# zju3dv/OnePose_Plus_Plus

Hardware: AMD Instinct MI355X
Metric: query images/sec (2D-3D match fwd) at 512x512 img x 5k pts (higher is better)
Workload: dtype f32 (operands as exact bf16 triples, f32 accumulate)

## Files before the change

### include/opp_hip.h

```cpp
#ifndef OPP_HIP_H
#define OPP_HIP_H

#include <stddef.h>

#ifdef __cplusplus
extern "C" {
#endif

#define OPP_MAX_LAYERS 16

typedef struct opp_config {
  int initial_dim;
  int block_dims[3];
  int kpt_enc_enable;
  int kpt_enc_dims[3];
  int pos_enc_enable;
  int coarse_d_model;
  int coarse_nhead;
  int coarse_n_layers;
  int coarse_is_cross[OPP_MAX_LAYERS];
  int fine_d_model;
  int fine_nhead;
  int fine_n_layers;
  int fine_is_cross[OPP_MAX_LAYERS];
// ... 31 lines not shown
                     size_t packed_bytes, void* stream);
int opp_set_pack_scope(opp_ctx* ctx, int scope);

int opp_num_bn_layers(const opp_ctx* ctx);
const char* opp_bn_layer_name(const opp_ctx* ctx, int i);
int opp_bn_layer_channels(const opp_ctx* ctx, int i);
size_t opp_packed_train_weights_bytes(const opp_ctx* ctx);
int opp_pack_train_weights(opp_ctx* ctx, const float* const* weights, int n_weights, void* packed,
                           size_t packed_bytes, void* stream);
size_t opp_backbone_train_workspace_bytes(const opp_ctx* ctx, int B, int H, int W);
int opp_backbone_train(opp_ctx* ctx, const float* image, int B, int H, int W, float* feat_c, float* feat_f,
                       float* bn_stats, void* workspace, size_t workspace_bytes, void* stream);

size_t opp_backbone_workspace_bytes(const opp_ctx* ctx, int H, int W);
int opp_backbone(opp_ctx* ctx, const float* image, int H, int W, float* feat_c, float* feat_f,
                 void* workspace, size_t workspace_bytes, void* stream);

int opp_coarse_tokens(opp_ctx* ctx, const float* feat_c, const float* pe, int L, const float* kpts,
                      const float* bank_c, int n_points, float* tokens, void* workspace,
                      size_t workspace_bytes, void* stream);

int opp_encode_points(opp_ctx* ctx, const float* kpts, const float* bank_c, int n_points,
                      float* tokens3d, void* workspace, size_t workspace_bytes, void* stream);

size_t opp_object_prefix_bytes(const opp_ctx* ctx, int n_points);
size_t opp_object_prefix_workspace_bytes(const opp_ctx* ctx, int n_points);
int opp_object_prefix(opp_ctx* ctx, const float* tokens3d, int n_points, void* prefix, size_t prefix_bytes, void* workspace,
                      size_t workspace_bytes, void* stream);
int opp_set_object_prefix(opp_ctx* ctx, const void* prefix, int n_points);

size_t opp_transformer_workspace_bytes(const opp_ctx* ctx, int which, int n_seg, int len0, int len1);
int opp_transformer(opp_ctx* ctx, int which, float* tokens, int n_seg, int len0, int len1,
                    void* workspace, size_t workspace_bytes, void* stream);

size_t opp_coarse_match_workspace_bytes(const opp_ctx* ctx, int n_points, int L);
int opp_coarse_match(opp_ctx* ctx, const float* feat3d, const float* feat2d, int n_points, int hc,
                     int wc, const float* kpts, float base_scale, const float* query_scale, float* conf,
                     long long* i_ids, long long* j_ids, float* mconf, float* mkpts_c,
                     float* mkpts_3d, int* count, void* workspace, size_t workspace_bytes,
                     void* stream);

size_t opp_forward_coarse_workspace_bytes(const opp_ctx* ctx, int H, int W, int n_points);
int opp_forward_coarse(opp_ctx* ctx, const float* image, int H, int W, const float* pe,
                       const float* kpts, const float* bank_c, const float* tokens3d_pre, int n_points,
                       float base_scale, const float* query_scale, float* feat_f, float* conf, long long* i_ids,
                       long long* j_ids, float* mconf, float* mkpts_c, float* mkpts_3d, int* count,
                       void* workspace, size_t workspace_bytes, void* stream);

size_t opp_fine_workspace_bytes(const opp_ctx* ctx, int n_matches);
int opp_fine(opp_ctx* ctx, const float* feat_f, int Hf, int Wf, const float* bank_f, int n_points,
             const long long* i_ids, const long long* j_ids, int n_matches, int hc, int wc,
             const float* mkpts_c, float base_scale, const float* query_scale, int run_transformer,
             float* expec_f, float* mkpts_f, void* workspace, size_t workspace_bytes, void* stream);

int opp_set_fine_patch_buffers(opp_ctx* ctx, float* x1, float* x2_out);
size_t opp_fine_patch_buffer_floats(const opp_ctx* ctx, int H, int W, int which);
size_t opp_fine_patches_workspace_bytes(const opp_ctx* ctx, int n_matches);
int opp_fine_patches(opp_ctx* ctx, const float* x1, const float* x2_out, int H, int W, const float* bank_f, int n_points,
                     const long long* i_ids, const long long* j_ids, int n_matches, int hc, int wc, const float* mkpts_c,
                     float base_scale, const float* query_scale, int run_transformer, float* expec_f, float* mkpts_f,
                     void* workspace, size_t workspace_bytes, void* stream);
size_t opp_backbone_fine_branch_workspace_bytes(const opp_ctx* ctx, int H, int W);
int opp_backbone_fine_branch(opp_ctx* ctx, const float* x1, const float* x2_out, int H, int W, float* feat_f, void* workspace,
                             size_t workspace_bytes, void* stream);

size_t opp_focal_loss_workspace_bytes(size_t n);
// ... 130 lines not shown
```

### onepose_plus_plus_amd/_lib.py

```python
import ctypes
import os
from ctypes import (POINTER, Structure, c_char_p, c_float, c_int, c_longlong, c_size_t, c_void_p)

_HERE = os.path.dirname(os.path.abspath(__file__))
LIB_PATH = os.environ.get("OPP_HIP_LIB") or os.path.join(_HERE, "libopp_hip.so")
OPP_MAX_LAYERS = 16


class OppConfig(Structure):
    _fields_ = [
        ("initial_dim", c_int),
        ("block_dims", c_int * 3),
        ("kpt_enc_enable", c_int),
        ("kpt_enc_dims", c_int * 3),
        ("pos_enc_enable", c_int),
        ("coarse_d_model", c_int),
        ("coarse_nhead", c_int),
        ("coarse_n_layers", c_int),
        ("coarse_is_cross", c_int * OPP_MAX_LAYERS),
        ("fine_d_model", c_int),
        ("fine_nhead", c_int),
        ("fine_n_layers", c_int),
        ("fine_is_cross", c_int * OPP_MAX_LAYERS),
        ("fine_window", c_int),
# ... 13 lines not shown
SIGNATURES = {
    "opp_last_error": (c_char_p, []),
    "opp_version": (c_int, []),
    "opp_source_hash": (c_char_p, []),
    "opp_supports_precision": (c_int, [c_int]),
    "opp_profile_event_overhead": (c_int, [c_int, POINTER(ctypes.c_double), c_void_p]),
    "opp_profile_empty_kernel": (c_int, [c_int, POINTER(ctypes.c_double), c_void_p]),
    "opp_profile_event_calibration": (c_int, [c_int, ctypes.c_double, POINTER(ctypes.c_double), POINTER(ctypes.c_double), c_void_p]),
    "opp_create": (c_int, [POINTER(OppConfig), POINTER(c_void_p)]),
    "opp_destroy": (None, [c_void_p]),
    "opp_set_status_flag": (c_int, [c_void_p, c_void_p]),
    "opp_set_query_mask": (c_int, [c_void_p, c_void_p]),
    "opp_set_conv_tail": (c_int, [c_void_p, c_int]),
    "opp_set_keypoint_extent_ref": (c_int, [c_void_p, c_void_p, c_int]),
    "opp_num_weights": (c_int, [c_void_p]),
    "opp_weight_name": (c_char_p, [c_void_p, c_int]),
    "opp_weight_numel": (c_longlong, [c_void_p, c_int]),
    "opp_num_bn_layers": (c_int, [c_void_p]),
    "opp_bn_layer_name": (c_char_p, [c_void_p, c_int]),
    "opp_bn_layer_channels": (c_int, [c_void_p, c_int]),
    "opp_packed_train_weights_bytes": (c_size_t, [c_void_p]),
    "opp_pack_train_weights": (c_int, [c_void_p, POINTER(c_void_p), c_int, c_void_p, c_size_t, c_void_p]),
    "opp_backbone_train_workspace_bytes": (c_size_t, [c_void_p, c_int, c_int, c_int]),
    "opp_backbone_train": (c_int, [c_void_p, c_void_p, c_int, c_int, c_int, c_void_p, c_void_p, c_void_p, c_void_p, c_size_t, c_void_p]),
    "opp_packed_weights_bytes": (c_size_t, [c_void_p]),
    "opp_set_pack_scope": (c_int, [c_void_p, c_int]),
    "opp_pack_weights": (c_int, [c_void_p, POINTER(c_void_p), c_int, c_void_p, c_size_t, c_void_p]),
    "opp_backbone_workspace_bytes": (c_size_t, [c_void_p, c_int, c_int]),
    "opp_backbone": (c_int, [c_void_p, c_void_p, c_int, c_int, c_void_p, c_void_p, c_void_p, c_size_t, c_void_p]),
    "opp_coarse_tokens": (c_int, [c_void_p, c_void_p, c_void_p, c_int, c_void_p, c_void_p, c_int, c_void_p,
                                  c_void_p, c_size_t, c_void_p]),
    "opp_transformer_workspace_bytes": (c_size_t, [c_void_p, c_int, c_int, c_int, c_int]),
    "opp_transformer": (c_int, [c_void_p, c_int, c_void_p, c_int, c_int, c_int, c_void_p, c_size_t, c_void_p]),
    "opp_coarse_match_workspace_bytes": (c_size_t, [c_void_p, c_int, c_int]),
    "opp_coarse_match": (c_int, [c_void_p, c_void_p, c_void_p, c_int, c_int, c_int, c_void_p, c_float, c_void_p,
                                 c_void_p, c_void_p, c_void_p, c_void_p, c_void_p, c_void_p, c_void_p,
                                 c_void_p, c_size_t, c_void_p]),
    "opp_forward_coarse_workspace_bytes": (c_size_t, [c_void_p, c_int, c_int, c_int]),
    "opp_encode_points": (c_int, [c_void_p, c_void_p, c_void_p, c_int, c_void_p, c_void_p, c_size_t, c_void_p]),
    "opp_object_prefix_bytes": (c_size_t, [c_void_p, c_int]),
    "opp_object_prefix_workspace_bytes": (c_size_t, [c_void_p, c_int]),
    "opp_object_prefix": (c_int, [c_void_p, c_void_p, c_int, c_void_p, c_size_t, c_void_p, c_size_t, c_void_p]),
    "opp_set_object_prefix": (c_int, [c_void_p, c_void_p, c_int]),
    "opp_forward_coarse": (c_int, [c_void_p, c_void_p, c_int, c_int, c_void_p, c_void_p, c_void_p, c_void_p, c_int, c_float,
                                   c_void_p, c_void_p, c_void_p, c_void_p, c_void_p, c_void_p, c_void_p,
                                   c_void_p, c_void_p, c_void_p, c_size_t, c_void_p]),
    "opp_fine_workspace_bytes": (c_size_t, [c_void_p, c_int]),
    "opp_fine_head_train_forward": (c_int, [c_void_p, c_void_p, c_int, c_int, c_int, c_void_p, c_void_p, c_void_p]),
    "opp_fine_head_train_backward": (c_int, [c_void_p, c_void_p, c_int, c_int, c_int, c_void_p, c_void_p, c_void_p, c_void_p]),
    "opp_build_assignmatrix": (c_int, [c_void_p, c_void_p, c_int, c_void_p, c_int, c_int, c_int, c_int, c_float, c_float, c_float, c_void_p, c_void_p,
                                       c_void_p, c_void_p, c_void_p]),
    "opp_set_fine_patch_buffers": (c_int, [c_void_p, c_void_p, c_void_p]),
    "opp_fine_patch_buffer_floats": (c_size_t, [c_void_p, c_int, c_int, c_int]),
    "opp_fine_patches_workspace_bytes": (c_size_t, [c_void_p, c_int]),
    "opp_fine_patches": (c_int, [c_void_p, c_void_p, c_void_p, c_int, c_int, c_void_p, c_int, c_void_p, c_void_p, c_int, c_int, c_int,
                                 c_void_p, c_float, c_void_p, c_int, c_void_p, c_void_p, c_void_p, c_size_t, c_void_p]),
    "opp_backbone_fine_branch_workspace_bytes": (c_size_t, [c_void_p, c_int, c_int]),
    "opp_backbone_fine_branch": (c_int, [c_void_p, c_void_p, c_void_p, c_int, c_int, c_void_p, c_void_p, c_size_t, c_void_p]),
    "opp_fine": (c_int, [c_void_p, c_void_p, c_int, c_int, c_void_p, c_int, c_void_p, c_void_p, c_int, c_int, c_int,
                         c_void_p, c_float, c_void_p, c_int, c_void_p, c_void_p, c_void_p, c_size_t, c_void_p]),
    "opp_conv2d_nhwc": (c_int, [c_void_p, c_int, c_int, c_int, c_void_p, c_void_p, c_int, c_int, c_int, c_void_p,
                                c_int, c_int, c_void_p, c_int, c_int, c_void_p, c_void_p]),
    "opp_conv2d_nhwc_split": (c_int, [c_void_p, c_void_p, c_int, c_int, c_int, c_void_p, c_void_p, c_int, c_int, c_int, c_void_p,
                                      c_int, c_int, c_void_p, c_void_p, c_int, c_void_p]),
    "opp_conv_packed_k": (c_int, [c_int, c_int]),
    "opp_dual_softmax_backward_workspace_bytes": (c_size_t, [c_int, c_int, c_int]),
# ... 99 lines not shown
```

### onepose_plus_plus_amd/csrc/api.hip

```cpp
#include <math.h>
#include <stdarg.h>

#include <string>
#include <vector>

#include "../../include/opp_hip.h"
#include "opp_internal.h"

static thread_local char g_err[512] = "";
void opp_set_error(const char* fmt, ...) {
  va_list ap;
  va_start(ap, fmt);
  vsnprintf(g_err, sizeof(g_err), fmt, ap);
  va_end(ap);
}
extern "C" const char* opp_last_error(void) { return g_err; }
extern "C" int opp_version(void) { return 1; }

namespace {

inline int pad32(int c) { return (c + 31) / 32 * 32; }

inline int gemm_prec(const opp_config& cfg) {
  return cfg.gemm_precision == 3 ? OPP_PREC_BF16X3 : cfg.gemm_precision ? OPP_PREC_FP16X2 : OPP_PREC_FP32;
// ... 1479 lines not shown
      ch.w1 = e.f1;
      ch.w2 = e.f2;
      ch.g1 = e.g1;
      ch.b1 = e.b1;
      ch.g2 = e.g2;
      ch.b2 = e.b2;
      ch.eps_ln = eps_ln;
      OPP_TRY(opp_enc_chain(ch, s));
      continue;
    }
    OPP_TRY(encoder_tail_dense(e, X, b, T, C, fuse_ln, eps_ln, s, h2));
  }
  return OPP_OK;
}

int transformer_impl(const std::vector<EncLayerDesc>& layers, const int* is_cross, int C, int nhead, float* X, int n_seg,
                     int len0, int len1, Arena& a, hipStream_t s, int h2, const float* mask0 = nullptr, int fusion = 1,
                     int prefix_mode = OPP_PREFIX_NONE, const ObjPrefix* pre = nullptr) {
  const int D = C / nhead;
  const int T0 = n_seg * len0, T1 = n_seg * len1, T = T0 + T1;
  if (T == 0 || layers.empty()) return OPP_OK;
  if (prefix_mode != OPP_PREFIX_NONE)
    OPP_CHECK_ARG(pre && n_seg == 1 && C == 256 && D == 32 && fusion == 2 && h2 == OPP_PREC_BF16X3 && layers.size() >= 2 && !is_cross[0] && is_cross[1] &&
                      (prefix_mode == OPP_PREFIX_USE || len0 == 0), "transformer: object prefix on an unsupported configuration");
  TrBufs b;
  plan_transformer(C, D, n_seg, len0, len1, a, b);
  if (!a.ok) {
    opp_set_error("transformer: workspace too small");
    return OPP_ERR_WORKSPACE;
  }
  const float eps_attn = 1e-6f, eps_ln = 1e-5f;
  static const int fuse_env = getenv("OPP_FUSE_LN") ? atoi(getenv("OPP_FUSE_LN")) : 1;
  const bool fuse_ln = fuse_env && (C == 256 || C == 128);
  for (size_t li = 0; li < layers.size(); ++li) {
    const EncLayerDesc& e = layers[li];
    const bool cross = is_cross[li] != 0;
    const int l1_qkv = (prefix_mode == OPP_PREFIX_USE && li < 2) ? 0 : len1;
    const int l1_lay = (prefix_mode == OPP_PREFIX_USE && li == 0) ? 0 : len1;
    const bool make_tail = prefix_mode == OPP_PREFIX_MAKE && li == 1;
    static const bool fold_env = !(getenv("OPP_QKV_FOLD") && getenv("OPP_QKV_FOLD")[0] == '0');
    const bool fold_path = fold_env && fusion == 2 && h2 == OPP_PREC_BF16X3 && n_seg == 1 && C == 256 && D == 32 && e.fmerge && e.fqkv;
    if (!(fold_path && li > 0)) {
      OppGemm g;
      g.nonfinite = t_status_flag;
      g.tile_policy = t_tile_policy;
      g.A0 = X;
      g.lda0 = C;
      g.ksplit = C;
      g.W = e.wqkv;
      g.ldw = (int)split_floats((size_t)C, h2);
      g.M = T0 + n_seg * l1_qkv;
      g.N = 3 * C;
      g.K = C;
      g.C = make_tail ? pre->qkv1 : b.qkv;
      g.ldc = 3 * C;
      g.n_store = 3 * C;
      g.act = OPP_ACT_QKV;
      g.qk_cols = 2 * C;
      g.split_row = T0;
      g.s0 = (float)len0;
      g.s1 = (float)len1;
      g.row_mask = mask0;
      g.row_mask_rows = T0;
      g.prec = h2;
      g.h2_inv = (h2 == OPP_PREC_FP16X2 && e.sqkv) ? e.sqkv + 1 : nullptr;
      OPP_TRY(opp_gemm_launch(g, s));
    }
    if (make_tail) {
      OPP_TRY(opp_linattn_kv_pair(pre->qkv1, 3 * C, 0, len1, b.kv, b.ks, b.scratch, s));
      OPP_TRY(copy_f(pre->kv1, b.kv + (size_t)C * D, (size_t)C * D, s));
      return copy_f(pre->ks1, b.ks + C, C, s);
    }
    const bool chain_apply = n_seg == 1 && C == 256 && D == 32;
    if (fusion && h2 == OPP_PREC_BF16X3 && e.fmerge && opp_enc_chain_ok(C, nhead, chain_apply)) {
      OPP_TRY(run_linattn(b.qkv, C, D, n_seg, len0, l1_qkv, cross, b.kv, b.ks, b.scratch, chain_apply ? nullptr : b.msg, eps_attn, s));
      OppEncChain ch;
      ch.C = C;
      ch.X = X;
      ch.ldx = C;
      ch.out = X;
      ch.ldo = C;
      ch.len0 = chain_apply ? len0 : T;
      ch.len1 = chain_apply ? l1_lay : 0;
      if (prefix_mode == OPP_PREFIX_USE && li == 1) {
        ch.q1 = pre->qkv1;
        ch.kv1 = pre->kv1;
        ch.ks1 = pre->ks1;
      }
      if (fold_path && li + 1 < layers.size() && layers[li + 1].fqkv) {
        ch.wq_next = layers[li + 1].fqkv;
        ch.qkv_out = b.qkv;
        ch.qkv_out1 = (prefix_mode == OPP_PREFIX_MAKE && li == 0) ? pre->qkv1 : nullptr;
        ch.qmask = mask0;
      }
      ch.msg = b.msg;
      ch.ldm = C;
      ch.apply = chain_apply ? 1 : 0;
      ch.q = b.qkv;
      ch.ldq = 3 * C;
      ch.kv = b.kv;
      ch.ks = b.ks;
      ch.cross = cross ? 1 : 0;
      ch.eps_attn = eps_attn;
      ch.wm = e.fmerge;
      ch.w1 = e.f1;
      ch.w2 = e.f2;
      ch.g1 = e.g1;
      ch.b1 = e.b1;
      ch.g2 = e.g2;
      ch.b2 = e.b2;
      ch.eps_ln = eps_ln;
      if (chain_apply && fusion == 2) OPP_TRY(opp_enc_layer64(ch, s));
      else OPP_TRY(opp_enc_chain(ch, s));
      continue;
    }
    OPP_TRY(run_linattn(b.qkv, C, D, n_seg, len0, len1, cross, b.kv, b.ks, b.scratch, b.msg, eps_attn, s));
    OPP_TRY(encoder_tail_dense(e, X, b, T, C, fuse_ln, eps_ln, s, h2));
  }
  return OPP_OK;
}

}

extern "C" int opp_coarse_tokens(opp_ctx* ctx, const float* feat_c, const float* pe, int L, const float* kpts,
                                 const float* bank_c, int n, float* tokens, void* ws, size_t ws_bytes, void* stream) {
  OPP_CHECK_ARG(ctx && ctx->packed && feat_c && kpts && bank_c && tokens && ws, "coarse_tokens: null argument");
// ... 68 lines not shown
  Arena a(ws, ws_bytes);
  float *kv, *ks, *sc;
  plan_linear_attention(C, C / nhead, n_seg, len0, len1, a, &kv, &ks, &sc);
  if (!a.ok) {
    opp_set_error("linear_attention: workspace too small");
    return OPP_ERR_WORKSPACE;
  }
  return run_linattn(qkv, C, C / nhead, n_seg, len0, len1, cross != 0, kv, ks, sc, msg, 1e-6f, (hipStream_t)stream);
}

extern "C" size_t opp_full_attention_workspace_bytes(int n_seg, int len0, int len1, int C, int nhead) {
  (void)n_seg, (void)len0, (void)len1, (void)C, (void)nhead;
  return 0;
}

extern "C" int opp_full_attention(const float* qkv, int n_seg, int len0, int len1, int C, int nhead, int cross, int precision, float* msg,
                                  void* ws, size_t ws_bytes, void* stream) {
  (void)ws, (void)ws_bytes;
  if (precision != 0 && precision != 3) {
    opp_set_error("full_attention: precision must be 0 (fp32) or 3 (bf16x3), got %d", precision);
    return OPP_ERR_UNSUPPORTED;
  }
  return opp_full_attention_run(qkv, n_seg, len0, len1, C, nhead, cross != 0, precision == 3 ? OPP_PREC_BF16X3 : OPP_PREC_FP32, msg,
                                (hipStream_t)stream);
}

extern "C" size_t opp_transformer_workspace_bytes(const opp_ctx* ctx, int which, int n_seg, int len0, int len1) {
  if (!ctx) return 0;
  const int C = which == 0 ? ctx->cfg.coarse_d_model : ctx->cfg.fine_d_model;
  const int nh = which == 0 ? ctx->cfg.coarse_nhead : ctx->cfg.fine_nhead;
  Arena a(nullptr, 0);
  TrBufs b;
  return opp_align(plan_transformer(C, C / nh, n_seg, len0, len1, a, b)) + 256;
}

extern "C" int opp_transformer(opp_ctx* ctx, int which, float* tokens, int n_seg, int len0, int len1, void* ws,
                               size_t ws_bytes, void* stream) {
  FlagScope flag_scope(ctx);
  OPP_CHECK_ARG(ctx && ctx->packed && tokens && ws, "transformer: null argument");
  OPP_CHECK_ARG(ctx->tr_packed, "transformer: weights were packed with scope 1 (backbone only); repack with opp_set_pack_scope(ctx, 0)");
  OPP_CHECK_ARG(which == 0 || which == 1, "transformer: which must be 0 or 1");
  Arena a(ws, ws_bytes);
  if (which == 0 && ctx->cfg.coarse_attention) {
    OPP_CHECK_ARG(n_seg != 1 || !ctx->query_mask, "transformer: full attention with a query mask is unsupported (upstream FullAttention indexes the "
                                                  "None q_mask of the cross layers, linear_attention.py:84-85)");
    return transformer_full_impl(ctx->coarse, ctx->cfg.coarse_is_cross, ctx->cfg.coarse_d_model, ctx->cfg.coarse_nhead, tokens, n_seg, len0, len1, a,
                                 (hipStream_t)stream, gemm_prec(ctx->cfg), ctx->cfg.encoder_fusion);
  }
  if (which == 1 && ctx->cfg.fine_attention)
    return transformer_full_impl(ctx->fine, ctx->cfg.fine_is_cross, ctx->cfg.fine_d_model, ctx->cfg.fine_nhead, tokens, n_seg, len0, len1, a,
                                 (hipStream_t)stream, gemm_prec(ctx->cfg), ctx->cfg.encoder_fusion);
  if (which == 0)
    return transformer_impl(ctx->coarse, ctx->cfg.coarse_is_cross, ctx->cfg.coarse_d_model, ctx->cfg.coarse_nhead, tokens, n_seg, len0, len1, a, (hipStream_t)stream, gemm_prec(ctx->cfg),
                            n_seg == 1 ? ctx->query_mask : nullptr, ctx->cfg.encoder_fusion);
  return transformer_impl(ctx->fine, ctx->cfg.fine_is_cross, ctx->cfg.fine_d_model, ctx->cfg.fine_nhead, tokens, n_seg, len0, len1, a, (hipStream_t)stream, gemm_prec(ctx->cfg),
                          nullptr, ctx->cfg.encoder_fusion);
}

namespace {

int coarse_match_impl(opp_ctx* c, const float* f3, const float* f2, int n, int hc, int wc, const float* kpts, float base_scale,
                      const float* qscale, float* conf, long long* i_ids, long long* j_ids, float* mconf, float* mkpts_c,
                      float* mkpts_3d, int* count, Arena& a, hipStream_t s) {
  const int C = c->cfg.coarse_d_model, L = hc * wc;
  float* scratch = a.f(opp_coarse_match_scratch_floats(n, L));
  float* stats = a.f(opp_coarse_match_stats_floats(n, L));
// ... 616 lines not shown
```

### onepose_plus_plus_amd/csrc/attention.hip

```cpp
#include "opp_internal.h"

namespace {

__device__ __forceinline__ float wave_sum(float v) {
#pragma unroll
  for (int o = 32; o > 0; o >>= 1) v += __shfl_xor(v, o, 64);
  return v;
}

template <int VPT>
__global__ __launch_bounds__(256) void layernorm_kernel(const float* __restrict__ x, int ldx,
                                                        const float* __restrict__ gamma,
                                                        const float* __restrict__ beta,
                                                        const float* __restrict__ res, int ldres,
                                                        float* __restrict__ out, int ldo, int rows,
                                                        float eps) {
  constexpr int RPW = 4;
  constexpr int C = 64 * VPT;
  const int lane = threadIdx.x & 63;
  const int row0 = (blockIdx.x * 4 + (threadIdx.x >> 6)) * RPW;
  if (row0 >= rows) return;
  float v[RPW][VPT], rv[RPW][VPT], gm[VPT], bt[VPT];
  typedef float vec_t __attribute__((ext_vector_type(VPT)));
  auto ldv = [](const float* p, float (&dst)[VPT]) {
// ... 295 lines not shown
  float ksum = 0.f;
  for (int s = s_begin; s < s_end; s += 16) {
    float kk[8], vv[8];
#pragma unroll
    for (int u = 0; u < 8; ++u) {
      const int t = s + 2 * u + half;
      const bool ok = t < s_end;
      kk[u] = ok ? kbase[(size_t)t * ld] : 0.f;
      vv[u] = ok ? vbase[(size_t)t * ld] : 0.f;
    }
#pragma unroll
    for (int u = 0; u < 8; ++u) {
      acc = __builtin_amdgcn_mfma_f32_32x32x2f32(kk[u], vv[u], acc, 0, 0, 0);
      ksum += kk[u];
    }
  }
#pragma unroll
  for (int r = 0; r < 16; ++r) {
    const int d = (r & 3) + 8 * (r >> 2) + 4 * half;
    acc_sh[wave][d * 32 + l31] = acc[r];
  }
  const float tot = ksum + __shfl_xor(ksum, 32, 64);
  if (half == 0) ks_sh[wave][l31] = tot;
  __syncthreads();
  float* kvp = kv_part + (size_t)grp * (C * 32) + h * 1024;
#pragma unroll
  for (int i = 0; i < 4; ++i) {
    const int o = threadIdx.x + i * 256;
    kvp[o] = (acc_sh[0][o] + acc_sh[1][o]) + (acc_sh[2][o] + acc_sh[3][o]);
  }
  if (threadIdx.x < 32) ks_part[(size_t)grp * C + h * 32 + threadIdx.x] = (ks_sh[0][threadIdx.x] + ks_sh[1][threadIdx.x]) + (ks_sh[2][threadIdx.x] + ks_sh[3][threadIdx.x]);
}

__global__ __launch_bounds__(256) void linattn_reduce_pair_kernel(const float* __restrict__ kv_part,
                                                                 const float* __restrict__ ks_part, int chunks0,
                                                                 int chunks1, float* __restrict__ out_kv,
                                                                 float* __restrict__ out_ks) {
  constexpr int KV = 8192, C = 256;
  __shared__ float red[4][64];
  const int stream = blockIdx.y;
  const int c_begin = stream ? chunks0 : 0;
  const int c_end = stream ? chunks0 + chunks1 : chunks0;
  const int e = threadIdx.x & 63, gq = threadIdx.x >> 6;
  const int i = blockIdx.x * 64 + e;
  float s = 0.f;
  if (i < KV) {
    for (int c = c_begin + gq; c < c_end; c += 4) s += kv_part[(size_t)c * KV + i];
  } else if (i < KV + C) {
    for (int c = c_begin + gq; c < c_end; c += 4) s += ks_part[(size_t)c * C + (i - KV)];
  }
  red[gq][e] = s;
  __syncthreads();
  if (gq == 0) {
    const float tot = ((red[0][e] + red[1][e]) + red[2][e]) + red[3][e];
    if (i < KV) out_kv[stream * KV + i] = tot;
    else if (i < KV + C) out_ks[stream * C + (i - KV)] = tot;
  }
}

constexpr int kApplyChunk = 32;
__global__ __launch_bounds__(512) void linattn_apply_pair_kernel(const float* __restrict__ qkv, int ld,
                                                                const float* __restrict__ kv,
                                                                const float* __restrict__ ks, int cross,
                                                                float* __restrict__ out, int ldo, int len0, int len1,
                                                                int chunks0, float eps) {
  constexpr int C = 256, D = 32, H = 8, CHUNK = kApplyChunk, QS = 258;
  __shared__ __attribute__((aligned(16))) float qsh[CHUNK * QS];
  __shared__ float z_sh[H][CHUNK];
  const int t = threadIdx.x;
  const int stream = blockIdx.x >= chunks0 ? 1 : 0;
  const int cidx = stream ? blockIdx.x - chunks0 : blockIdx.x;
  const int seg_len = stream ? len1 : len0;
  const int base = stream ? len0 : 0;
  const int src = cross ? 1 - stream : stream;
  const float src_len = (float)(src ? len1 : len0);
  const int s_begin = cidx * CHUNK;
  const float* kvp = kv + (size_t)src * (C * D);
  const float* ksp = ks + (size_t)src * C;
  const int lane = t & 63, h = t >> 6;
  const int half = lane >> 5, l31 = lane & 31;
  float bk[16];
#pragma unroll
// ... 107 lines not shown
bool opp_linattn_small_ok(int len0, int len1, int C, int D) {
  return C == 128 && D == 16 && len0 > 0 && len1 > 0 && len0 + len1 <= 32;
}

int opp_linattn_small_pair(const float* qkv, int ld, int n_seg, int len0, int len1, int cross, float* out, int ldo, int C, int D,
                           float eps, hipStream_t stream) {
  if (n_seg <= 0) return OPP_OK;
  OPP_CHECK_ARG(opp_linattn_small_ok(len0, len1, C, D) && ld % 4 == 0, "linattn_small_pair: unsupported shape");
  const size_t lds = ((size_t)(len0 + len1) * 2 * C + 2 * C + (size_t)(len0 + len1) * (C / D)) * sizeof(float);
  OppProfScope prof(OPP_PROF_LINATTN_SMALL, stream, (double)n_seg * (len0 + len1) * C * 4.0 * 4.0);
  hipLaunchKernelGGL((linattn_small_pair_kernel<16, 128>), dim3(n_seg), dim3(128), lds, stream, qkv, ld, n_seg, len0, len1, cross, out,
                     ldo, eps);
  OPP_CHECK_LAUNCH("linattn_small_pair_kernel");
  return OPP_OK;
}

size_t opp_linattn_pair_scratch_floats(int len0, int len1) {
  const size_t chunks = (size_t)opp_cdiv(len0, kPairChunk) + opp_cdiv(len1, kPairChunk);
  return chunks * (8192 + 256);
}

int opp_linattn_kv_pair(const float* qkv, int ld, int len0, int len1, float* kv, float* ks, float* scratch,
                        hipStream_t stream) {
  const int c0 = opp_cdiv(opp_cdiv(len0, kPairChunk), kPairGroup), c1 = opp_cdiv(opp_cdiv(len1, kPairChunk), kPairGroup);
  float* kvp = scratch;
  float* ksp = scratch + (size_t)(c0 + c1) * 8192;
  if (c0 + c1 == 0) return OPP_OK;
  {
    OppProfScope prof(OPP_PROF_LINATTN_KV, stream, (double)(len0 + len1) * 512.0 * 4.0 + (double)(c0 + c1) * (8192 + 256) * 4.0);
    hipLaunchKernelGGL(linattn_kv_mfma_kernel, dim3(c0 + c1, 8), dim3(256), 0, stream, qkv, ld, len0, len1, c0, kvp, ksp);
  }
  {
    OppProfScope prof(OPP_PROF_LINATTN_REDUCE, stream, (double)(c0 + c1 + 2) * (8192 + 256) * 4.0);
    hipLaunchKernelGGL(linattn_reduce_pair_kernel, dim3(opp_cdiv(8192 + 256, 64), 2), dim3(256), 0, stream, kvp, ksp, c0, c1, kv, ks);
  }
  OPP_CHECK_LAUNCH("linattn_kv_pair");
  return OPP_OK;
}

int opp_linattn_apply_pair(const float* qkv, int ld, const float* kv, const float* ks, int cross, float* out, int ldo,
                           int len0, int len1, float eps, hipStream_t stream) {
  const int c0 = opp_cdiv(len0, kApplyChunk), c1 = opp_cdiv(len1, kApplyChunk);
  OppProfScope prof(OPP_PROF_LINATTN_APPLY, stream, (double)(len0 + len1) * 256.0 * 4.0 * 2.0);
  hipLaunchKernelGGL(linattn_apply_pair_kernel, dim3(c0 + c1), dim3(512), 0, stream, qkv, ld, kv, ks, cross, out, ldo, len0, len1,
                     c0, eps);
  OPP_CHECK_LAUNCH("linattn_apply_pair_kernel");
  return OPP_OK;
}
```

### onepose_plus_plus_amd/csrc/enc_layer64.hip

```cpp
#include <stdlib.h>

#include <type_traits>

#include "enc_frag.h"

namespace {

constexpr int R64 = 64, C = 256, NW = 8, NT = 512, D = 32;
constexpr int SA = a_stride_bytes(C);
constexpr int SS = C + 4;
constexpr int OFF_S = R64 * SA, OFF_Z = OFF_S + 32 * SS * 4;
constexpr size_t kLds64 = OFF_Z + 1024;

__global__ __launch_bounds__(NT) void enc_layer64_kernel(const OppEncChain a) {
  extern __shared__ __attribute__((aligned(16))) char smem[];
  char* A = smem;
  float* S = reinterpret_cast<float*>(smem + OFF_S);
  float* z_sh = reinterpret_cast<float*>(smem + OFF_Z);

  const int tid = threadIdx.x, lane = tid & 63;
  const int wave = __builtin_amdgcn_readfirstlane(tid >> 6);
  const int half = lane >> 5, l31 = lane & 31;

  const int chunks0 = (a.len0 + R64 - 1) / R64;
  const int stream = (int)blockIdx.x >= chunks0 ? 1 : 0;
  const int cidx = stream ? blockIdx.x - chunks0 : blockIdx.x;
  const int seg_len = stream ? a.len1 : a.len0;
  const int row0 = (stream ? a.len0 : 0) + cidx * R64;
  const int nrows = min(R64, seg_len - cidx * R64);
  const float* qrows = (stream && a.q1 != nullptr) ? a.q1 + (size_t)(cidx * R64) * a.ldq : a.q + (size_t)row0 * a.ldq;

  const char* a_lane = A + l31 * SA + half * 48;
  auto gemm = [&](auto ntile_c, auto depth_c, auto s0_c, auto s1_c, auto ks_c, const void* wf, int t0, f32x16 (&acc)[2][decltype(ntile_c)::value]) {
    constexpr int NTILE = decltype(ntile_c)::value, DEPTH = decltype(depth_c)::value;
    constexpr int S0 = decltype(s0_c)::value, S1 = decltype(s1_c)::value, KS = decltype(ks_c)::value;
    constexpr int NSTEP = S1 - S0;
    const __amdgpu_buffer_rsrc_t rsrc = __builtin_amdgcn_make_buffer_rsrc(const_cast<void*>(wf), 0, 0x7fffffff, 0x00020000);
    const int voff = lane * 16;
    u32x4 bq[DEPTH][NTILE][3];
    u32x4 af[2][2][3];
    auto load_b = [&](int s, int slot) {
#pragma unroll
      for (int j = 0; j < NTILE; ++j)
#pragma unroll
        for (int p = 0; p < 3; ++p)
          bq[slot][j][p] = __builtin_amdgcn_raw_buffer_load_b128(rsrc, voff, (((t0 + j) * KS + S0 + s) * 3 + p) * 1024, 0);
    };
    auto load_a = [&](int s, int slot) {
#pragma unroll
      for (int i = 0; i < 2; ++i)
#pragma unroll
        for (int q = 0; q < 3; ++q) af[slot][i][q] = *reinterpret_cast<const u32x4*>(a_lane + i * 32 * SA + s * 96 + q * 16);
    };
#pragma unroll
    for (int s = 0; s < DEPTH && s < NSTEP; ++s) load_b(s, s);
    load_a(0, 0);
    __builtin_amdgcn_sched_barrier(0);
    constexpr int PA[6] = {2, 0, 1, 1, 0, 0};
    constexpr int PB[6] = {0, 2, 1, 0, 1, 0};
#pragma unroll
    for (int s = 0; s < NSTEP; ++s) {
      if (s + 1 < NSTEP) load_a(s + 1, (s + 1) & 1);
#pragma unroll
      for (int pr = 0; pr < 6; ++pr)
#pragma unroll
        for (int i = 0; i < 2; ++i)
#pragma unroll
          for (int j = 0; j < NTILE; ++j)
            acc[i][j] = __builtin_amdgcn_mfma_f32_32x32x16_bf16(__builtin_bit_cast(bf16x8, af[s & 1][i][PA[pr]]),
                                                                 __builtin_bit_cast(bf16x8, bq[s % DEPTH][j][PB[pr]]), acc[i][j], 0, 0, 0);
      if (s + DEPTH < NSTEP) load_b(s + DEPTH, s % DEPTH);
      __builtin_amdgcn_sched_barrier(0);
    }
  };
  auto ic = [](auto v) { return v; };
  (void)ic;
  auto stage = [&](const f32x16& t, int col0, bool relu) {
#pragma unroll
    for (int r = 0; r < 16; ++r) {
// ... 187 lines not shown
  f32x16 out[2][1];
  zero2(out);
#pragma unroll
  for (int kh = 0; kh < 2; ++kh) {
#pragma unroll
    for (int rh = 0; rh < 2; ++rh) {
      if (wave / (NW / 2) == kh) {
        const int c0 = (wave - kh * (NW / 2)) * 64;
        stage(hid[rh][0], c0, true);
        stage(hid[rh][1], c0 + 32, true);
      }
      __syncthreads();
      split_staged(rh * 32, 0);
      __syncthreads();
    }
    if (kh == 0) gemm(I1{}, I4{}, I0{}, I16{}, I32{}, a.w2, wave, out);
    else gemm(I1{}, I4{}, I16{}, I32{}, I32{}, a.w2, wave, out);
    __syncthreads();
  }

  const bool fold = a.wq_next != nullptr;
#pragma unroll
  for (int rh = 0; rh < 2; ++rh) {
    stage(out[rh][0], wave * 32, false);
    __syncthreads();
    if (fold) layernorm_rows(a.g2, a.b2, a.eps_ln, I2{}, rh * 32);
    else layernorm_rows(a.g2, a.b2, a.eps_ln, I1{}, rh * 32);
    __syncthreads();
  }
  if (!fold) return;

  float* qdst = (stream && a.qkv_out1 != nullptr) ? a.qkv_out1 + (size_t)(cidx * R64) * (3 * C) : a.qkv_out + (size_t)row0 * (3 * C);
  const float vdiv = (float)seg_len;
  auto store_qkv = [&](const f32x16& t, int rb, int tile) {
    const int col = tile * 32 + l31;
#pragma unroll
    for (int r = 0; r < 16; ++r) {
      const int row = rb + (r & 3) + 8 * (r >> 2) + 4 * half;
      if (row < nrows) {
        float v = t[r];
        if (col < 2 * C) v = v > 0.f ? v + 1.f : __expf(v);
        else v = v / vdiv;
        if (stream == 0 && a.qmask != nullptr) v *= a.qmask[row0 + row];
        qdst[(size_t)row * (3 * C) + col] = v;
      }
    }
  };
  {
    f32x16 acc[2][2];
    zero2(acc);
    gemm(I2{}, I3{}, I0{}, I16{}, I16{}, a.wq_next, wave * 3, acc);
#pragma unroll
    for (int i = 0; i < 2; ++i)
#pragma unroll
      for (int j = 0; j < 2; ++j) store_qkv(acc[i][j], i * 32, wave * 3 + j);
  }
  {
    f32x16 acc[2][1];
    zero2(acc);
    gemm(I1{}, I4{}, I0{}, I16{}, I16{}, a.wq_next, wave * 3 + 2, acc);
#pragma unroll
    for (int i = 0; i < 2; ++i) store_qkv(acc[i][0], i * 32, wave * 3 + 2);
  }
}

}

int opp_enc_layer64(const OppEncChain& a, hipStream_t stream) {
  OPP_CHECK_ARG(a.C == 256 && a.apply && a.X && a.out && a.q && a.kv && a.ks && a.wm && a.w1 && a.w2 && a.g1 && a.b1 && a.g2 && a.b2,
                "enc_layer64: coarse level (C = 256) with the fused attention apply only");
  OPP_CHECK_ARG(a.len0 >= 0 && a.len1 >= 0 && a.len0 + a.len1 > 0, "enc_layer64: empty token set");
  auto al16 = [](const void* p) { return (reinterpret_cast<uintptr_t>(p) & 15) == 0; };
  OPP_CHECK_ARG(al16(a.X) && al16(a.out) && al16(a.q) && a.ldx % 4 == 0 && a.ldo % 4 == 0 && a.ldq % 4 == 0 && al16(a.g1) && al16(a.b1) &&
                    al16(a.g2) && al16(a.b2) && al16(a.wm) && al16(a.w1) && al16(a.w2) && al16(a.q1), "enc_layer64: operands must be 16-byte aligned");
  OPP_CHECK_ARG(a.wq_next == nullptr || (a.qkv_out != nullptr && al16(a.wq_next)), "enc_layer64: folded projection needs its output buffer");
  static OppLdsOnce lds_once;
  opp_lds_opt_in(reinterpret_cast<const void*>(enc_layer64_kernel), kLds64, lds_once);
  const int tiles = opp_cdiv(a.len0, R64) + opp_cdiv(a.len1, R64);
  OppProfScope prof(OPP_PROF_ENC_CHAIN, stream, 2.0 * (double)(a.len0 + a.len1) * ((a.wq_next ? 10.0 : 7.0) * C * C + 32.0 * C));
  hipLaunchKernelGGL(enc_layer64_kernel, dim3(tiles), dim3(NT), kLds64, stream, a);
  OPP_CHECK_LAUNCH("enc_layer64_kernel");
  return OPP_OK;
}
```

### onepose_plus_plus_amd/csrc/opp_internal.h

```cpp
#pragma once
#include "opp_common.h"

enum {
  OPP_PROF_FIRST_NON_GEMM = 1000,
  OPP_PROF_LINATTN_KV = 1000,
  OPP_PROF_LINATTN_APPLY = 1001,
  OPP_PROF_CONF = 1002,
  OPP_PROF_FINE = 1003,
  OPP_PROF_LINATTN_SMALL = 1004,
  OPP_PROF_FINE_GATHER = 1005,
  OPP_PROF_FINE_HEAD = 1006,
  OPP_PROF_FOCAL_FWD = 1007,
  OPP_PROF_FOCAL_BWD = 1008,
  OPP_PROF_ENC_CHAIN = 1009,
  OPP_PROF_SCORE_SWEEP1 = 1010,
  OPP_PROF_SCORE_SWEEP2 = 1011,
  OPP_PROF_CONV_WGRAD = 1013,
  OPP_PROF_CONV_SPLITK = 1014,
  OPP_PROF_CONV_TAIL = 1017,
  OPP_PROF_LINATTN_REDUCE = 1016,
  OPP_PROF_SPLITK_EPILOGUE = 1015,
  OPP_PROF_SCORE_SS = 1012,
};
inline int opp_prof_gemm_symbol(int tile_cfg, int kind) { return kind * 256 + tile_cfg; }
struct OppProfScope {
  OppProfScope(int symbol, hipStream_t stream, double work);
  ~OppProfScope();
  OppProfScope(const OppProfScope&) = delete;
  OppProfScope& operator=(const OppProfScope&) = delete;

 private:
  hipStream_t stream_;
  long long slot_ = -1;
};

int opp_layernorm(const float* x, int ldx, const float* gamma, const float* beta, const float* res, int ldres,
                  float* out, int ldo, int rows, int C, float eps, hipStream_t stream);
int opp_linattn_chunks(int seg_len);
int opp_linattn_kv(const float* k, const float* v, int ld, int n_seg, int seg_len, int C, int D, float* kv_out,
                   float* ks_out, float* scratch, hipStream_t stream);
int opp_linattn_apply(const float* q, int ldq, const float* kv, const float* ks, float* out, int ldo, int n_seg,
                      int seg_len, int src_len, int C, int D, float eps, hipStream_t stream);
size_t opp_linattn_pair_scratch_floats(int len0, int len1);
int opp_linattn_kv_pair(const float* qkv, int ld, int len0, int len1, float* kv, float* ks, float* scratch,
                        hipStream_t stream);
size_t opp_focal_loss_ws_bytes(size_t n);
int opp_focal_loss_fwd(const float* conf, const short* gt, const float* weight, size_t n, float alpha, float gamma, double* sums,
                       void* ws, size_t ws_bytes, hipStream_t stream);
int opp_focal_loss_bwd(const float* conf, const short* gt, const float* weight, size_t n, float alpha, float gamma,
                       const float* scales, float* grad, hipStream_t stream);
int opp_focal_loss_fwd_ex(const float* conf, const void* gt, int gt_kind, const float* weight, const float* mask0, const float* mask1, int N, int L,
                          size_t n, float alpha, float gamma, double* sums, void* ws, size_t ws_bytes, hipStream_t stream);
int opp_focal_loss_bwd_ex(const float* conf, const void* gt, int gt_kind, const float* weight, const float* mask0, const float* mask1, int N, int L,
                          size_t n, float alpha, float gamma, const float* scales, float* grad, hipStream_t stream);
size_t opp_dual_softmax_bwd_ws_bytes(int B, int N, int L);
int opp_dual_softmax_bwd(const float* g, const float* sim, const float* lse_row, const float* lse_col, int B, int N, int L, float* ds,
                         void* ws, size_t ws_bytes, hipStream_t stream);
bool opp_linattn_small_ok(int len0, int len1, int C, int D);
int opp_full_attention_run(const float* qkv, int n_seg, int len0, int len1, int C, int nhead, int cross, int prec, float* msg,
                           hipStream_t stream);
int opp_linattn_small_pair(const float* qkv, int ld, int n_seg, int len0, int len1, int cross, float* out, int ldo, int C, int D,
                           float eps, hipStream_t stream);
int opp_linattn_apply_pair(const float* qkv, int ld, const float* kv, const float* ks, int cross, float* out, int ldo,
                           int len0, int len1, float eps, hipStream_t stream);
struct OppEncChain {
  int C = 256;
  const float* X = nullptr;
  int ldx = 0;
  float* out = nullptr;
  int ldo = 0;
  int len0 = 0, len1 = 0;
  const float* msg = nullptr;
  int ldm = 0;
  int apply = 0;
  const float* q = nullptr;
  int ldq = 0;
  const float* kv = nullptr;
  const float* ks = nullptr;
  const float* q1 = nullptr;
  const float* kv1 = nullptr;
  const float* ks1 = nullptr;
  const void* wq_next = nullptr;
  float* qkv_out = nullptr;
  float* qkv_out1 = nullptr;
  const float* qmask = nullptr;
  int cross = 0;
  float eps_attn = 1e-6f;
  const void* wm = nullptr;
  const void* w1 = nullptr;
  const void* w2 = nullptr;
  const float *g1 = nullptr, *b1 = nullptr, *g2 = nullptr, *b2 = nullptr;
  float eps_ln = 1e-5f;
};
size_t opp_frag_b3_bytes(int N, int K);
int opp_pack_frag_b3(const float* w, int N, int K, void* out, hipStream_t stream);
bool opp_enc_chain_ok(int C, int nhead, bool apply);
int opp_enc_chain(const OppEncChain& a, hipStream_t stream);
int opp_enc_layer64(const OppEncChain& a, hipStream_t stream);
enum { OPP_SS_STATS = 1, OPP_SS_CONF = 2, OPP_SS_STATS_STORE = 3 };
struct OppGemmSS {
  const void* A = nullptr;
  const void* B = nullptr;
  int lda = 0, ldb = 0;
  int M = 0, N = 0, K = 0;
  int mode = OPP_SS_STATS;
  float out_mul = 1.f, out_div = 1.f;
  const float* row_mask = nullptr;
  float* stat_rowmax = nullptr;
  float* stat_rowsum = nullptr;
  float* stat_colmax = nullptr;
  float* stat_colsum = nullptr;
  const float* rstat_max = nullptr;
  const float* rstat_sum = nullptr;
  const float* cstat_max = nullptr;
  const float* cstat_sum = nullptr;
  float* C = nullptr;
  int ldc = 0;
  float* part_best = nullptr;
// ... 95 lines not shown
```

Measured before the change: 562.7.

## Fold linear-attention KV partial sums into the fused encoder layer epilogue

The fused 64-row encoder layer kernel now computes the next layer's K^T V and K-sum partials per tile directly from its freshly projected K and V registers using MFMA and lane swaps. The next layer then only runs a chunk-reduction kernel instead of the full KV pass. The tile-to-wave assignment of the QKV projection is reshuffled so each wave holds matching K and V columns for one head, and the K/V stores to global memory are skipped when folding. This removes a separate read of the QKV buffer and one kernel launch per layer, at the cost of heavier epilogue register pressure and an added reduction step.

```diff
diff --git a/include/opp_hip.h b/include/opp_hip.h
--- a/include/opp_hip.h
+++ b/include/opp_hip.h
@@ -87,6 +87,7 @@
 size_t opp_transformer_workspace_bytes(const opp_ctx* ctx, int which, int n_seg, int len0, int len1);
 int opp_transformer(opp_ctx* ctx, int which, float* tokens, int n_seg, int len0, int len1,
                     void* workspace, size_t workspace_bytes, void* stream);
+int opp_transformer_kv_offsets(const opp_ctx* ctx, int which, int n_seg, int len0, int len1, size_t* kv_offset, size_t* ks_offset);
 
 size_t opp_coarse_match_workspace_bytes(const opp_ctx* ctx, int n_points, int L);
 int opp_coarse_match(opp_ctx* ctx, const float* feat3d, const float* feat2d, int n_points, int hc,
diff --git a/onepose_plus_plus_amd/_lib.py b/onepose_plus_plus_amd/_lib.py
--- a/onepose_plus_plus_amd/_lib.py
+++ b/onepose_plus_plus_amd/_lib.py
@@ -69,6 +69,7 @@
                                   c_void_p, c_size_t, c_void_p]),
     "opp_transformer_workspace_bytes": (c_size_t, [c_void_p, c_int, c_int, c_int, c_int]),
     "opp_transformer": (c_int, [c_void_p, c_int, c_void_p, c_int, c_int, c_int, c_void_p, c_size_t, c_void_p]),
+    "opp_transformer_kv_offsets": (c_int, [c_void_p, c_int, c_int, c_int, c_int, POINTER(c_size_t), POINTER(c_size_t)]),
     "opp_coarse_match_workspace_bytes": (c_size_t, [c_void_p, c_int, c_int]),
     "opp_coarse_match": (c_int, [c_void_p, c_void_p, c_void_p, c_int, c_int, c_int, c_void_p, c_float, c_void_p,
                                  c_void_p, c_void_p, c_void_p, c_void_p, c_void_p, c_void_p, c_void_p,
diff --git a/onepose_plus_plus_amd/csrc/api.hip b/onepose_plus_plus_amd/csrc/api.hip
--- a/onepose_plus_plus_amd/csrc/api.hip
+++ b/onepose_plus_plus_amd/csrc/api.hip
@@ -1535,6 +1535,8 @@
   const float eps_attn = 1e-6f, eps_ln = 1e-5f;
   static const int fuse_env = getenv("OPP_FUSE_LN") ? atoi(getenv("OPP_FUSE_LN")) : 1;
   const bool fuse_ln = fuse_env && (C == 256 || C == 128);
+  const bool kv_fold_env = !(getenv("OPP_KV_FOLD") && getenv("OPP_KV_FOLD")[0] == '0');
+  bool kv_parts = false;
   for (size_t li = 0; li < layers.size(); ++li) {
     const EncLayerDesc& e = layers[li];
     const bool cross = is_cross[li] != 0;
@@ -1576,7 +1578,9 @@
     }
     const bool chain_apply = n_seg == 1 && C == 256 && D == 32;
     if (fusion && h2 == OPP_PREC_BF16X3 && e.fmerge && opp_enc_chain_ok(C, nhead, chain_apply)) {
-      OPP_TRY(run_linattn(b.qkv, C, D, n_seg, len0, l1_qkv, cross, b.kv, b.ks, b.scratch, chain_apply ? nullptr : b.msg, eps_attn, s));
+      if (kv_parts) OPP_TRY(opp_linattn_reduce_chunks(len0, l1_qkv, b.kv, b.ks, b.scratch, s));
+      else OPP_TRY(run_linattn(b.qkv, C, D, n_seg, len0, l1_qkv, cross, b.kv, b.ks, b.scratch, chain_apply ? nullptr : b.msg, eps_attn, s));
+      kv_parts = false;
       OppEncChain ch;
       ch.C = C;
       ch.X = X;
@@ -1595,6 +1599,11 @@
         ch.qkv_out = b.qkv;
         ch.qkv_out1 = (prefix_mode == OPP_PREFIX_MAKE && li == 0) ? pre->qkv1 : nullptr;
         ch.qmask = mask0;
+        const int l1_next = (prefix_mode == OPP_PREFIX_USE && li + 1 < 2) ? 0 : len1;
+        if (kv_fold_env && chain_apply && fusion == 2 && prefix_mode != OPP_PREFIX_MAKE && layers[li + 1].fmerge && ch.len1 == l1_next) {
+          opp_linattn_chunk_parts(b.scratch, ch.len0, ch.len1, &ch.kv_part, &ch.ks_part);
+          kv_parts = true;
+        }
       }
       ch.msg = b.msg;
       ch.ldm = C;
@@ -1729,6 +1738,19 @@
   Arena a(nullptr, 0);
   TrBufs b;
   return opp_align(plan_transformer(C, C / nh, n_seg, len0, len1, a, b)) + 256;
+}
+
+extern "C" int opp_transformer_kv_offsets(const opp_ctx* ctx, int which, int n_seg, int len0, int len1, size_t* kv_offset, size_t* ks_offset) {
+  OPP_CHECK_ARG(ctx && kv_offset && ks_offset && (which == 0 || which == 1), "transformer_kv_offsets: bad argument");
+  const int C = which == 0 ? ctx->cfg.coarse_d_model : ctx->cfg.fine_d_model;
+  const int nh = which == 0 ? ctx->cfg.coarse_nhead : ctx->cfg.fine_nhead;
+  char* const base = reinterpret_cast<char*>(uintptr_t(1) << 20);
+  Arena a(base, ~size_t(0) >> 1);
+  TrBufs b;
+  plan_transformer(C, C / nh, n_seg, len0, len1, a, b);
+  *kv_offset = (size_t)(reinterpret_cast<char*>(b.kv) - base);
+  *ks_offset = (size_t)(reinterpret_cast<char*>(b.ks) - base);
+  return OPP_OK;
 }
 
 extern "C" int opp_transformer(opp_ctx* ctx, int which, float* tokens, int n_seg, int len0, int len1, void* ws,
diff --git a/onepose_plus_plus_amd/csrc/attention.hip b/onepose_plus_plus_amd/csrc/attention.hip
--- a/onepose_plus_plus_amd/csrc/attention.hip
+++ b/onepose_plus_plus_amd/csrc/attention.hip
@@ -351,22 +351,32 @@
   if (threadIdx.x < 32) ks_part[(size_t)grp * C + h * 32 + threadIdx.x] = (ks_sh[0][threadIdx.x] + ks_sh[1][threadIdx.x]) + (ks_sh[2][threadIdx.x] + ks_sh[3][threadIdx.x]);
 }
 
+template <bool PER_CHUNK>
 __global__ __launch_bounds__(256) void linattn_reduce_pair_kernel(const float* __restrict__ kv_part,
-                                                                 const float* __restrict__ ks_part, int chunks0,
-                                                                 int chunks1, float* __restrict__ out_kv,
+                                                                 const float* __restrict__ ks_part, int n0,
+                                                                 int n1, float* __restrict__ out_kv,
                                                                  float* __restrict__ out_ks) {
   constexpr int KV = 8192, C = 256;
   __shared__ float red[4][64];
   const int stream = blockIdx.y;
-  const int c_begin = stream ? chunks0 : 0;
-  const int c_end = stream ? chunks0 + chunks1 : chunks0;
+  const int c_begin = stream ? n0 : 0;
+  const int c_end = stream ? n0 + n1 : n0;
   const int e = threadIdx.x & 63, gq = threadIdx.x >> 6;
   const int i = blockIdx.x * 64 + e;
+  const float* part = i < KV ? kv_part + i : ks_part + (i - KV);
+  const size_t width = i < KV ? KV : C;
   float s = 0.f;
-  if (i < KV) {
-    for (int c = c_begin + gq; c < c_end; c += 4) s += kv_part[(size_t)c * KV + i];
-  } else if (i < KV + C) {
-    for (int c = c_begin + gq; c < c_end; c += 4) s += ks_part[(size_t)c * C + (i - KV)];
+  if (i < KV + C) {
+    if constexpr (PER_CHUNK) {
+      for (int c = c_begin + gq * kPairGroup; c < c_end; c += 4 * kPairGroup) {
+        float p[kPairGroup];
+#pragma unroll
+        for (int w = 0; w < kPairGroup; ++w) p[w] = c + w < c_end ? part[(size_t)(c + w) * width] : 0.f;
+        s += (p[0] + p[1]) + (p[2] + p[3]);
+      }
+    } else {
+      for (int c = c_begin + gq; c < c_end; c += 4) s += part[(size_t)c * width];
+    }
   }
   red[gq][e] = s;
   __syncthreads();
@@ -540,9 +550,26 @@
   }
   {
     OppProfScope prof(OPP_PROF_LINATTN_REDUCE, stream, (double)(c0 + c1 + 2) * (8192 + 256) * 4.0);
-    hipLaunchKernelGGL(linattn_reduce_pair_kernel, dim3(opp_cdiv(8192 + 256, 64), 2), dim3(256), 0, stream, kvp, ksp, c0, c1, kv, ks);
+    hipLaunchKernelGGL(linattn_reduce_pair_kernel<false>, dim3(opp_cdiv(8192 + 256, 64), 2), dim3(256), 0, stream, kvp, ksp, c0, c1, kv, ks);
   }
   OPP_CHECK_LAUNCH("linattn_kv_pair");
+  return OPP_OK;
+}
+
+void opp_linattn_chunk_parts(float* scratch, int len0, int len1, float** kv_part, float** ks_part) {
+  const size_t chunks = (size_t)opp_cdiv(len0, kPairChunk) + opp_cdiv(len1, kPairChunk);
+  *kv_part = scratch;
+  *ks_part = scratch + chunks * 8192;
+}
+
+int opp_linattn_reduce_chunks(int len0, int len1, float* kv, float* ks, float* scratch, hipStream_t stream) {
+  const int c0 = opp_cdiv(len0, kPairChunk), c1 = opp_cdiv(len1, kPairChunk);
+  if (c0 + c1 == 0) return OPP_OK;
+  float *kvp, *ksp;
+  opp_linattn_chunk_parts(scratch, len0, len1, &kvp, &ksp);
+  OppProfScope prof(OPP_PROF_LINATTN_REDUCE, stream, (double)(c0 + c1 + 2) * (8192 + 256) * 4.0);
+  hipLaunchKernelGGL(linattn_reduce_pair_kernel<true>, dim3(opp_cdiv(8192 + 256, 64), 2), dim3(256), 0, stream, kvp, ksp, c0, c1, kv, ks);
+  OPP_CHECK_LAUNCH("linattn_reduce_pair_kernel");
   return OPP_OK;
 }
 
diff --git a/onepose_plus_plus_amd/csrc/enc_layer64.hip b/onepose_plus_plus_amd/csrc/enc_layer64.hip
--- a/onepose_plus_plus_amd/csrc/enc_layer64.hip
+++ b/onepose_plus_plus_amd/csrc/enc_layer64.hip
@@ -31,7 +31,7 @@
   const float* qrows = (stream && a.q1 != nullptr) ? a.q1 + (size_t)(cidx * R64) * a.ldq : a.q + (size_t)row0 * a.ldq;
 
   const char* a_lane = A + l31 * SA + half * 48;
-  auto gemm = [&](auto ntile_c, auto depth_c, auto s0_c, auto s1_c, auto ks_c, const void* wf, int t0, f32x16 (&acc)[2][decltype(ntile_c)::value]) {
+  auto gemm = [&](auto ntile_c, auto depth_c, auto s0_c, auto s1_c, auto ks_c, const void* wf, int t0, f32x16 (&acc)[2][decltype(ntile_c)::value], int tstep = 1) {
     constexpr int NTILE = decltype(ntile_c)::value, DEPTH = decltype(depth_c)::value;
     constexpr int S0 = decltype(s0_c)::value, S1 = decltype(s1_c)::value, KS = decltype(ks_c)::value;
     constexpr int NSTEP = S1 - S0;
@@ -44,7 +44,7 @@
       for (int j = 0; j < NTILE; ++j)
 #pragma unroll
         for (int p = 0; p < 3; ++p)
-          bq[slot][j][p] = __builtin_amdgcn_raw_buffer_load_b128(rsrc, voff, (((t0 + j) * KS + S0 + s) * 3 + p) * 1024, 0);
+          bq[slot][j][p] = __builtin_amdgcn_raw_buffer_load_b128(rsrc, voff, (((t0 + j * tstep) * KS + S0 + s) * 3 + p) * 1024, 0);
     };
     auto load_a = [&](int s, int slot) {
 #pragma unroll
@@ -298,35 +298,91 @@
 
   float* qdst = (stream && a.qkv_out1 != nullptr) ? a.qkv_out1 + (size_t)(cidx * R64) * (3 * C) : a.qkv_out + (size_t)row0 * (3 * C);
   const float vdiv = (float)seg_len;
+  auto finish_qkv = [&](f32x16& t, int rb, bool qk) {
+#pragma unroll
+    for (int r = 0; r < 16; ++r) {
+      const int row = rb + (r & 3) + 8 * (r >> 2) + 4 * half;
+      float v = 0.f;
+      if (row < nrows) {
+        v = t[r];
+        if (qk) v = v > 0.f ? v + 1.f : __expf(v);
+        else v = v / vdiv;
+        if (stream == 0 && a.qmask != nullptr) v *= a.qmask[row0 + row];
+      }
+      t[r] = v;
+    }
+  };
   auto store_qkv = [&](const f32x16& t, int rb, int tile) {
     const int col = tile * 32 + l31;
 #pragma unroll
     for (int r = 0; r < 16; ++r) {
       const int row = rb + (r & 3) + 8 * (r >> 2) + 4 * half;
-      if (row < nrows) {
-        float v = t[r];
-        if (col < 2 * C) v = v > 0.f ? v + 1.f : __expf(v);
-        else v = v / vdiv;
-        if (stream == 0 && a.qmask != nullptr) v *= a.qmask[row0 + row];
-        qdst[(size_t)row * (3 * C) + col] = v;
-      }
-    }
-  };
-  {
-    f32x16 acc[2][2];
-    zero2(acc);
-    gemm(I2{}, I3{}, I0{}, I16{}, I16{}, a.wq_next, wave * 3, acc);
-#pragma unroll
-    for (int i = 0; i < 2; ++i)
-#pragma unroll
-      for (int j = 0; j < 2; ++j) store_qkv(acc[i][j], i * 32, wave * 3 + j);
-  }
+      if (row < nrows) qdst[(size_t)row * (3 * C) + col] = t[r];
+    }
+  };
+  const bool kv_fold = a.kv_part != nullptr;
   {
     f32x16 acc[2][1];
     zero2(acc);
-    gemm(I1{}, I4{}, I0{}, I16{}, I16{}, a.wq_next, wave * 3 + 2, acc);
-#pragma unroll
-    for (int i = 0; i < 2; ++i) store_qkv(acc[i][0], i * 32, wave * 3 + 2);
+    gemm(I1{}, I4{}, I0{}, I16{}, I16{}, a.wq_next, h, acc);
+#pragma unroll
+    for (int i = 0; i < 2; ++i) {
+      finish_qkv(acc[i][0], i * 32, true);
+      store_qkv(acc[i][0], i * 32, h);
+    }
+  }
+  f32x16 acc[2][2];
+  zero2(acc);
+  gemm(I2{}, I3{}, I0{}, I16{}, I16{}, a.wq_next, NW + h, acc, NW);
+#pragma unroll
+  for (int i = 0; i < 2; ++i) {
+    finish_qkv(acc[i][0], i * 32, true);
+    finish_qkv(acc[i][1], i * 32, false);
+  }
+  if (!kv_fold) {
+#pragma unroll
+    for (int i = 0; i < 2; ++i) {
+      store_qkv(acc[i][0], i * 32, NW + h);
+      store_qkv(acc[i][1], i * 32, 2 * NW + h);
+    }
+    return;
+  }
+  {
+    f32x16 kvacc;
+#pragma unroll
+    for (int r = 0; r < 16; ++r) kvacc[r] = 0.f;
+    float ksum = 0.f;
+    auto swap = [](float x, float y, float& lo, float& hi) {
+      const auto r = __builtin_amdgcn_permlane32_swap(__builtin_bit_cast(unsigned, x), __builtin_bit_cast(unsigned, y), false, false);
+      lo = __builtin_bit_cast(float, (unsigned)r[0]);
+      hi = __builtin_bit_cast(float, (unsigned)r[1]);
+    };
+#pragma unroll
+    for (int i = 0; i < 2; ++i)
+#pragma unroll
+      for (int q = 0; q < 4; ++q) {
+        float kk[2][2], vv[2][2];
+#pragma unroll
+        for (int e = 0; e < 2; ++e) {
+          swap(acc[i][0][4 * q + 2 * e], acc[i][0][4 * q + 2 * e + 1], kk[0][e], kk[1][e]);
+          swap(acc[i][1][4 * q + 2 * e], acc[i][1][4 * q + 2 * e + 1], vv[0][e], vv[1][e]);
+        }
+#pragma unroll
+        for (int g = 0; g < 2; ++g)
+#pragma unroll
+          for (int e = 0; e < 2; ++e) {
+            kvacc = __builtin_amdgcn_mfma_f32_32x32x2f32(kk[g][e], vv[g][e], kvacc, 0, 0, 0);
+            ksum += kk[g][e];
+          }
+      }
+    float* kvp = a.kv_part + (size_t)blockIdx.x * (C * D) + h * (D * D);
+#pragma unroll
+    for (int r = 0; r < 16; ++r) {
+      const int d = (r & 3) + 8 * (r >> 2) + 4 * half;
+      kvp[d * D + l31] = kvacc[r];
+    }
+    const float tot = ksum + __shfl_xor(ksum, 32, 64);
+    if (half == 0) a.ks_part[(size_t)blockIdx.x * C + h * D + l31] = tot;
   }
 }
 
@@ -340,6 +396,8 @@
   OPP_CHECK_ARG(al16(a.X) && al16(a.out) && al16(a.q) && a.ldx % 4 == 0 && a.ldo % 4 == 0 && a.ldq % 4 == 0 && al16(a.g1) && al16(a.b1) &&
                     al16(a.g2) && al16(a.b2) && al16(a.wm) && al16(a.w1) && al16(a.w2) && al16(a.q1), "enc_layer64: operands must be 16-byte aligned");
   OPP_CHECK_ARG(a.wq_next == nullptr || (a.qkv_out != nullptr && al16(a.wq_next)), "enc_layer64: folded projection needs its output buffer");
+  OPP_CHECK_ARG((a.kv_part == nullptr) == (a.ks_part == nullptr) && (a.kv_part == nullptr || (a.wq_next != nullptr && a.qkv_out1 == nullptr)),
+                "enc_layer64: the KV partials need the folded projection and both of their buffers");
   static OppLdsOnce lds_once;
   opp_lds_opt_in(reinterpret_cast<const void*>(enc_layer64_kernel), kLds64, lds_once);
   const int tiles = opp_cdiv(a.len0, R64) + opp_cdiv(a.len1, R64);
diff --git a/onepose_plus_plus_amd/csrc/opp_internal.h b/onepose_plus_plus_amd/csrc/opp_internal.h
--- a/onepose_plus_plus_amd/csrc/opp_internal.h
+++ b/onepose_plus_plus_amd/csrc/opp_internal.h
@@ -44,6 +44,8 @@
 size_t opp_linattn_pair_scratch_floats(int len0, int len1);
 int opp_linattn_kv_pair(const float* qkv, int ld, int len0, int len1, float* kv, float* ks, float* scratch,
                         hipStream_t stream);
+void opp_linattn_chunk_parts(float* scratch, int len0, int len1, float** kv_part, float** ks_part);
+int opp_linattn_reduce_chunks(int len0, int len1, float* kv, float* ks, float* scratch, hipStream_t stream);
 size_t opp_focal_loss_ws_bytes(size_t n);
 int opp_focal_loss_fwd(const float* conf, const short* gt, const float* weight, size_t n, float alpha, float gamma, double* sums,
                        void* ws, size_t ws_bytes, hipStream_t stream);
@@ -84,6 +86,8 @@
   float* qkv_out = nullptr;
   float* qkv_out1 = nullptr;
   const float* qmask = nullptr;
+  float* kv_part = nullptr;
+  float* ks_part = nullptr;
   int cross = 0;
   float eps_attn = 1e-6f;
   const void* wm = nullptr;
```

Result: faster. 572.5, median of 6 (+1.7%).
